# crockwell/far

Measured on AMD Instinct MI355X. Metric: image-pairs/sec (match+solve+regress) at 640x480, higher is better.
Workload: dtype f32

## Files before the change

far_amd/_lib.py:

```python
import ctypes
import os

from . import flags

_HERE = os.path.dirname(os.path.abspath(__file__))
LIB_PATH = flags.value('FAR_HIP_LIB') or os.path.join(_HERE, 'lib', 'libfar_hip.so')

c_p = ctypes.c_void_p
c_i = ctypes.c_int
c_f = ctypes.c_float
c_d = ctypes.c_double
c_sz = ctypes.c_size_t
c_l = ctypes.c_long
c_u32 = ctypes.c_uint32

SIGNATURES = {
    'far_abi_version': (c_i, []),
    'far_last_hip_error': (c_i, []),
    'far_set_tuning': (c_i, [c_i, c_i]),
    'far_mfma_probe_f16': (c_i, [c_i, c_i, c_i, c_p, c_p, c_p]),
    'far_dual_softmax_workspace_bytes': (c_sz, [c_i, c_i, c_i]),
    'far_dual_softmax_stats_f32': (c_i, [c_p, c_p, c_i, c_i, c_i, c_i, c_f, c_f, c_f, c_p, c_p, c_p, c_p, c_p, c_p]),
    'far_coarse_match_f32': (c_i, [c_p, c_p, c_i, c_i, c_i, c_i, c_f, c_f, c_i, c_i, c_i, c_i, c_i, c_f,
                                   c_p, c_p, c_p, c_p, c_p, c_p, c_p, c_p, c_p, c_p, c_p, c_p, c_p, c_p, c_p, c_p]),
# ... 24 lines not shown
    'far_sinkhorn_dense_focal_workspace_bytes': (c_sz, [c_i, c_i, c_i, c_i, c_i, c_i]),
    'far_sinkhorn_dense_focal_f16s': (c_i, [c_p, c_p, c_i, c_i, c_i, c_i, c_p, c_i, c_p, c_p, c_p, c_p, c_p, c_i, c_f, c_f, c_f, c_f,
                                            c_i, c_p, c_p, c_p, c_p]),
    'far_sinkhorn_dense_focal_bwd_f16': (c_i, [c_p, c_p, c_i, c_i, c_i, c_i, c_p, c_i, c_p, c_p, c_p, c_p, c_p, c_i, c_f, c_f, c_f, c_f,
                                               c_i, c_p, c_p, c_p, c_p, c_p, c_p]),
    'far_emm_pv_f32': (c_i, [c_p, c_p, c_p, c_p, c_i, c_i, c_i, c_f, c_p, c_p, c_p, c_p]),
    'far_fine_gather_f32': (c_i, [c_p, c_l, c_l, c_l, c_l, c_i, c_i, c_i, c_p, c_p, c_i, c_i, c_i, c_i, c_p, c_p]),
    'far_fine_scatter_f32': (c_i, [c_p, c_l, c_l, c_l, c_l, c_i, c_i, c_i, c_p, c_p, c_i, c_i, c_i, c_i, c_p, c_p]),
    'far_fine_scatter_det_f32': (c_i, [c_p, c_l, c_l, c_l, c_l, c_i, c_i, c_i, c_p, c_p, c_i, c_i, c_i, c_i, c_i, c_i, c_p, c_p]),
    'far_fine_expect_f32': (c_i, [c_p, c_p, c_i, c_i, c_i, c_p, c_f, c_p, c_p, c_p, c_p, c_p]),
    'far_linear_attention_workspace_bytes': (c_sz, [c_i, c_i, c_i, c_i]),
    'far_linear_attention_f32': (c_i, [c_p, c_p, c_p, c_i, c_i, c_i, c_i, c_i, c_p, c_p, c_f, c_p, c_p, c_p]),
    'far_linear_attention_apply_f32': (c_i, [c_p, c_p, c_i, c_i, c_i, c_i, c_p, c_f, c_p, c_p]),
    'far_full_attention_workspace_bytes': (c_sz, [c_i, c_i, c_i, c_i, c_i]),
    'far_full_attention_f16s': (c_i, [c_p, c_p, c_p, c_i, c_i, c_i, c_i, c_i, c_p, c_p, c_i, c_p, c_p, c_p, c_p]),
    'far_full_attention_train_f16s': (c_i, [c_p, c_p, c_p, c_i, c_i, c_i, c_i, c_i, c_p, c_p, c_i, c_p, c_p, c_p, c_p, c_p]),
    'far_full_attention_bwd_workspace_bytes': (c_sz, [c_i, c_i, c_i, c_i, c_i]),
    'far_full_attention_bwd_f16s': (c_i, [c_p, c_p, c_p, c_p, c_p, c_p, c_i, c_i, c_i, c_i, c_i, c_p, c_p, c_i, c_p, c_p, c_p, c_p, c_p, c_p]),
    'far_vit_attention_f16s': (c_i, [c_p, c_p, c_p, c_i, c_i, c_i, c_i, c_i, c_l, c_l, c_l, c_l, c_l, c_l, c_i, c_p, c_p, c_p]),
    'far_vit_attention_f16': (c_i, [c_p, c_p, c_p, c_i, c_i, c_i, c_i, c_i, c_l, c_l, c_l, c_l, c_l, c_l, c_i, c_p, c_p, c_p]),
    'far_vit_attention_train_f16s': (c_i, [c_p, c_p, c_p, c_i, c_i, c_i, c_i, c_i, c_l, c_l, c_l, c_l, c_l, c_l, c_i, c_p, c_p, c_p, c_p]),
    'far_vit_attention_bwd_workspace_bytes': (c_sz, [c_i, c_i, c_i, c_i, c_i]),
    'far_vit_attention_bwd_f16s': (c_i, [c_p] * 6 + [c_i] * 5 + [c_l] * 6 + [c_i, c_p, c_p, c_p] + [c_l] * 6 + [c_p, c_p, c_p]),
    'far_linear_attention_bwd_workspace_bytes': (c_sz, [c_i, c_i, c_i, c_i, c_i]),
    'far_linear_attention_bwd_f32': (c_i, [c_p, c_p, c_p, c_p, c_i, c_i, c_i, c_i, c_i, c_p, c_p, c_f, c_p, c_p, c_p, c_p, c_p]),
    'far_layernorm_f32': (c_i, [c_p, c_p, c_p, c_p, c_l, c_i, c_f, c_p, c_p]),
    'far_layernorm_bwd_ws_bytes': (c_l, [c_l, c_i]),
    'far_layernorm_bwd_f32': (c_i, [c_p, c_p, c_p, c_l, c_i, c_f, c_p, c_p, c_p, c_p, c_l, c_p]),
    'far_attn_block_packed_bytes': (c_sz, [c_i]),
    'far_attn_block_f16s': (c_i, [c_p, c_p, c_p, c_l, c_i, c_i, c_i, c_i, c_f, c_f, c_f, c_f, c_f, c_p, c_p, c_f, c_p, c_p, c_p]),
    'far_mlp_fused_packed_bytes': (c_sz, [c_i]),
    'far_mlp_fused_f16s': (c_i, [c_p, c_p, c_p, c_l, c_i, c_f, c_f, c_p, c_p, c_f, c_p, c_p, c_p]),
    'far_mlp_fused_f16': (c_i, [c_p, c_p, c_p, c_l, c_i, c_f, c_f, c_p, c_p, c_f, c_p, c_p, c_p]),
    'far_attn_block_f16': (c_i, [c_p, c_p, c_p, c_l, c_i, c_i, c_i, c_i, c_f, c_f, c_f, c_f, c_f, c_p, c_p, c_f, c_p, c_p, c_p]),
    'far_affine_act_f32': (c_i, [c_p, c_p, c_p, c_p, c_l, c_i, c_l, c_i, c_i, c_f, c_p, c_p]),
    'far_upsample2x_add_f32': (c_i, [c_p, c_p, c_i, c_i, c_i, c_i, c_i, c_p, c_p]),
    'far_upsample2x_bwd_f32': (c_i, [c_p, c_i, c_i, c_i, c_i, c_p, c_p]),
    'far_adamw_table_bytes': (c_l, [c_i, c_l]),
    'far_adamw_step_f32': (c_i, [c_p, c_i, c_l] + [ctypes.c_double] * 7 + [c_p]),
    'far_grad_norm_workspace_bytes': (c_sz, [c_l]),
    'far_grad_norm_f32': (c_i, [c_p, c_i, c_l, c_l, c_l, c_d, c_d, c_i, c_p, c_p]),
    'far_grad_clip_scale_f32': (c_i, [c_p, c_i, c_l, c_p, c_p]),
    'far_adam_step_f32': (c_i, [c_p, c_i, c_l] + [c_d] * 7 + [c_i, c_p, c_i, c_p]),
    'far_prior_from_pose_f32': (c_i, [c_p, c_p, c_p, c_i, c_p, c_p]),
    'far_bn_train_ws_bytes': (c_l, [c_l, c_i]),
    'far_bn_act_train_fwd_f32': (c_i, [c_p, c_p, c_l, c_i, c_p, c_p, c_f, c_f, c_p, c_p, c_i, c_f, c_p, c_p, c_p, c_l, c_p]),
    'far_bn_train_stats_f32': (c_i, [c_p, c_l, c_i, c_p, c_p, c_f, c_f, c_p, c_p, c_p, c_p, c_p, c_p, c_p, c_l, c_p]),
    'far_bn_train_bwd_f32': (c_i, [c_p, c_p, c_p, c_p, c_p, c_p, c_l, c_i, c_i, c_f, c_p, c_p, c_p, c_p, c_p, c_l, c_p]),
    'far_bn_sync_moments_f32': (c_i, [c_p, c_l, c_i, c_p, c_p, c_l, c_p]),
    'far_bn_sync_stats_f32': (c_i, [c_p, c_i, c_i, c_p, c_p, c_f, c_f, c_p, c_p, c_p, c_p]),
    'far_bn_sync_apply_f32': (c_i, [c_p, c_p, c_l, c_i, c_p, c_i, c_f, c_p, c_p]),
    'far_bn_sync_bwd_sums_f32': (c_i, [c_p, c_p, c_p, c_p, c_l, c_i, c_i, c_f, c_p, c_p, c_p, c_p, c_l, c_p]),
    'far_bn_sync_bwd_dx_f32': (c_i, [c_p, c_p, c_p, c_p, c_p, c_p, c_i, c_l, c_i, c_i, c_f, c_p, c_p, c_p, c_p]),
    'far_conv_packed_bytes': (c_sz, [c_i, c_i, c_i, c_i, c_i]),
    'far_conv_pack_f32': (c_i, [c_p, c_i, c_i, c_i, c_i, c_i, c_i, c_p, c_p]),
    'far_weight_scale_f32': (c_i, [c_p, c_l, c_p, c_p]),
    'far_conv_pack_view_f32': (c_i, [c_p, c_l, c_l, c_l, c_i, c_i, c_i, c_i, c_i, c_p, c_p, c_p]),
    'far_enc_layer_saved_floats': (c_l, [c_p]),
    'far_enc_layer_grads_floats': (c_l, [c_p]),
    'far_enc_layer_fwd_ws_bytes': (c_l, [c_p]),
    'far_enc_layer_bwd_ws_bytes': (c_l, [c_p]),
    'far_enc_layer_grads_offsets': (c_i, [c_p, c_p]),
    'far_enc_layer_fwd': (c_i, [c_p, c_p, c_p, c_p, c_p, c_p, c_l, c_p]),
    'far_enc_layer_bwd': (c_i, [c_p, c_p, c_p, c_p, c_p, c_p, c_p, c_l, c_p]),
    'far_stream_fork': (c_p, [c_p, c_i]),
    'far_stream_join': (c_i, [c_p, c_i]),
# ... 133 lines not shown
```

far_amd/flags.py:

```python
import os
from collections import namedtuple

Switch = namedtuple('Switch', 'env module attr off_value neutral scope doc')
SWITCHES = [
    Switch('FAR_NO_WINO', 'far_amd.ops', 'USE_WINO', False, 'parity', 'inference',
           'stride-1 3x3 convolutions on K9 (direct implicit GEMM) instead of K17 (Winograd F(2x2,3x3)); same operator, other summation'),
    Switch('FAR_NO_PAD', 'far_amd.loftr.backbone', 'PAD_CHANNELS', False, 'bitwise', 'inference',
           'the 196-channel backbone maps stored with 196 channels instead of 208 (zero weights for the extra ones: exact zeros)'),
    Switch('FAR_NO_PREFETCH', 'far_amd.loftr.model:LoFTR', 'head_prefetch', False, 'bitwise', 'inference',
           "the head's feature stage computed inside forward_rt_prediction instead of enqueued behind K1"),
    Switch('FAR_NO_SIDE_STREAM', 'far_amd.loftr.model:LoFTR', 'head_side_stream', False, 'bitwise', 'inference',
           "the head's feature stage on the step's own stream behind K1 (rounds 2-5) instead of on a second stream next to K1 and the fine level"),
    Switch('FAR_FPN_STREAM', 'far_amd.loftr.model:LoFTR', 'fpn_side_stream', True, 'bitwise', 'inference',
           "OPT-IN (1 switches it ON; default off): the FPN's fine branch on a side stream next to the coarse transformer and K1 (-0.6 ms per 32 "
           "pairs; off by default because the roofline launch -- K17 208 -> 208 @ 240x320 -- then shares the GPU and its in-step duration "
           "in a kernel trace is no longer its own)"),
    Switch('FAR_NO_GATHER_FUSE', 'far_amd.loftr.stages:FinePreprocess', 'fused_gather', False, 'bitwise', 'inference',
           'FinePreprocess.merge_feat on a materialised window tensor (K3 gather + K9) instead of K9 reading through the match indices'),
    Switch('FAR_NO_KV', 'far_amd.loftr.transformer:LoFTREncoderLayer', 'fused_kv', False, 'parity', 'inference',
           "k, v projections + K5's first half as separate launches instead of K9's k|v epilogue (the K'^T V sum changes order)"),
    Switch('FAR_NO_QAPPLY', 'far_amd.loftr.transformer:LoFTREncoderLayer', 'fused_apply', False, 'parity', 'inference',
           "q projection + K5's second half as separate launches instead of K9's attention-apply epilogue (q no longer stays in split operands)"),
    Switch('FAR_NO_STACK', 'far_amd.loftr.transformer:LocalFeatureTransformer', 'stack_self', False, 'bitwise', 'inference',
           "the two 'self' calls of an encoder layer on the two images separately instead of one call on both"),
    Switch('FAR_NO_BN', 'far_amd.ops', 'USE_HIP_BATCHNORM_TRAIN', False, 'parity', 'training',
           'training-mode BatchNorm on nn.BatchNorm2d + torch activations instead of K19 (tests/test_train_kernels_gpu.py holds K19 to the module)'),
]

ENV_ONLY = {
    'FAR_HIP_LIB': ('load', 'path of another build of libfar_hip.so (tools/ab_build.py: same-box A/B against a git revision); skips the build-id check'),
    'FAR_TUNING': ('load', 'comma-separated key=value pairs handed to far_set_tuning at load time, e.g. FAR_TUNING="10=1,8=1" (keys below)'),
    'FAR_SKIP_ASM_CHECK': ('build', "1: far_amd/build.py does not scan the generated code (K9's asm pixel loads; the LDS-DMA ring rule of every kernel with global_load_lds; the half-register writes of the asm fp16 split) after recompiling"),
    'FAR_EXTRA_HIPCC_FLAGS': ('build', 'extra hipcc flags of an experiment build (-DFAR_WINO_EXP=..., tools/wino_exp.sh); part of the build id'),
    'FAR_COMMIT': ('tools', 'commit stamp tools/collect_profiles.sh / tools/step_floors.py write into the profile files'),
    'FAR_C3_PY_NODE': ('bench', "bench.py --workload c3: the encoder layer's autograd node driven from Python instead of far_enc_layer_fwd / _bwd"),
    'FAR_C3_NO_OVERLAP': ('bench', 'bench.py --workload c3: the layer node without side streams'),
    'FAR_C3_PER_OP': ('bench', 'bench.py --workload c3: one autograd node per operator instead of per layer'),
    'FAR_TORCH_ADAMW': ('bench', 'bench.py --workload c3: torch.optim.AdamW instead of K20'),
    'FAR_CUDNN_BENCHMARK': ('bench', 'bench.py: torch.backends.cudnn.benchmark for the vendor comparison legs'),
}

Tuning = namedtuple('Tuning', 'key default values neutral doc')
TUNING = [
    Tuning(0, 3, (0, 1, 2, 4, 7), 'bitwise', 'bit mask of exact-f32 kernels that stagger wave-slot priorities: 1 k_stats, 2 k_match, 4 k_emm_pv'),
    Tuning(1, 0, (1,), 'parity', 'K1 exact-f32 variant: the other tile shape (another summation order of the row statistics)'),
    Tuning(2, 0, (1,), 'bitwise', 'conf_matrix writer variant A (store pattern)'),
    Tuning(3, 0, (1,), 'bitwise', 'conf_matrix writer variant B (store pattern)'),
    Tuning(4, 0, (1,), 'bitwise', 'K9 without the seven-tile mode / K5 windows on the generic path'),
    Tuning(5, 0, (1, 2, 4), 'bitwise', 'K5 apply: tiles per unit'),
    Tuning(6, 0, (64, 256), 'parity', "K5: tokens per K'^T V chunk (another partial-sum grouping)"),
    Tuning(7, 0, (1,), 'bitwise', 'K9 Linear launches always on full-height tiles'),
    Tuning(8, 0, (1,), 'bitwise', 'K17 splits its operands with the five-instruction split2 instead of v_fma_mix (same values)'),
    Tuning(9, 0, (1,), 'bitwise', 'K17 runs a short last channel block on the full body'),
    Tuning(10, 0, (1,), 'bitwise', "K1's match pass without the tile prescreen"),
    Tuning(11, 0, (1, 2), 'bitwise', "K14's pipeline: 0 = 4 waves / 3 slots / counted waits, two workgroups per CU; 1 = 8 waves / 4 slots / counted, one per CU (round 5's form); 2 = 4 waves / 3 slots / vmcnt(0) per phase (fallback without a wait table)"),
# ... 33 lines not shown
```

far_amd/loftr/transformer.py:

```python
import copy
import os
from functools import partial

import torch
import torch.nn as nn

from .. import _vendor as ag
from .. import flags, ops
from ..pose6d import pose_mean_6d, pose_std_6d


class LinearAttention(nn.Module):

    def __init__(self, eps=1e-6, use_num_corres=False):
        super().__init__()
        self.eps = eps
        self.use_num_corres = use_num_corres

    def forward(self, queries, keys, values, q_mask=None, kv_mask=None, loftr_preds=None):
        N, L, H, D = queries.shape
        S = keys.shape[1]
        if ag.needs_grad(queries, keys, values):
            if queries.is_cuda and D in (16, 32):
                return ops.linear_attention_train(queries.reshape(N, L, H * D), keys.reshape(N, S, H * D),
# ... 12 lines not shown

    def __init__(self, use_dropout=False, attention_dropout=0.1, use_num_corres=False):
        super().__init__()
        self.use_dropout = use_dropout
        self.attention_dropout = attention_dropout
        self.use_num_corres = use_num_corres

    def forward(self, queries, keys, values, q_mask=None, kv_mask=None, loftr_preds=None):
        N, L, H, D = queries.shape
        S = keys.shape[1]
        if self.training and self.use_dropout:
            raise NotImplementedError('FullAttention: dropout inside the softmax attention core is not built')
        if ag.needs_grad(queries, keys, values):
            if not self.full_training:
                raise NotImplementedError('FullAttention: training / gradients through the softmax attention core are off for this '
                                          'module (inference only); LoFTR.set_full_attention_training() / full_training = True '
                                          'turns the HIP backward on')
            return ops.full_attention_train(queries.reshape(N, L, H * D), keys.reshape(N, S, H * D), values.reshape(N, S, H * D), H,
                                            q_mask, kv_mask).view(N, L, H, D)
        out = ops.full_attention(queries.reshape(N, L, H * D).contiguous(), keys.reshape(N, S, H * D).contiguous(),
                                 values.reshape(N, S, H * D).contiguous(), H, q_mask, kv_mask)
        return out.view(N, L, H, D)


class LoFTREncoderLayer(nn.Module):
    split_operands = True
    dense_split = True
    hip_training = True
    full_training = False
    layer_node = True
    overlap = True
    native_node = True
    fused_mlp = True
    fused_attn = True
    fused_apply = not flags.off('FAR_NO_QAPPLY')
    fused_kv = not flags.off('FAR_NO_KV')

    def __init__(self, d_model, nhead, attention='linear', use_num_corres=False):
        super().__init__()
        if attention not in ('linear', 'full'):
            raise NotImplementedError(f"attention={attention!r}: only 'linear' (the FAR configuration) and 'full' have kernels")
        self.full = attention == 'full'
        self.dim = d_model // nhead
        self.nhead = nhead
        self.q_proj = nn.Linear(d_model, d_model, bias=False)
        self.k_proj = nn.Linear(d_model, d_model, bias=False)
        self.v_proj = nn.Linear(d_model, d_model, bias=False)
        self.attention = FullAttention(use_num_corres=use_num_corres) if self.full else LinearAttention(use_num_corres=use_num_corres)
        self.merge = nn.Linear(d_model, d_model, bias=False)
        self.mlp = nn.Sequential(
            nn.Linear(d_model * 2, d_model * 2, bias=False),
            nn.ReLU(True),
            nn.Linear(d_model * 2, d_model, bias=False),
        )
        self.norm1 = nn.LayerNorm(d_model)
        self.norm2 = nn.LayerNorm(d_model)

    def forward(self, x, source, x_mask=None, source_mask=None, loftr_preds=None, out=None):
        bs = x.size(0)
        if self.full and x.is_cuda and ag.needs_grad(x, source, self.norm1.weight) and not self.full_training:
            raise NotImplementedError("LoFTREncoderLayer(attention='full'): training / gradients through the softmax attention core "
                                      'are off for this layer (inference only); LoFTR.set_full_attention_training() / '
                                      'full_training = True turns the HIP backward on')
        if self.full and not x.is_cuda:
            raise ops._lib.FarHipError("LoFTREncoderLayer(attention='full') needs tensors on the GPU (no CPU fallback exists)")
        if ag.needs_grad(x, source, self.norm1.weight) or not x.is_cuda:
# ... 36 lines not shown
            h = ops.linear_f16s(x, lin('mlp0', self.mlp[0]), act='relu', x2=msg)
            return ops.linear_f16s(h, lin('mlp2', self.mlp[2]), ln=(self.norm2.weight, self.norm2.bias, self.norm2.eps),
                                   post_residual=x, out=out)
        if (not self.full and self.fused_kv and x.shape[-1] == 256 and self.nhead == 8 and source.shape[1] >= 64 and x_mask is None
                and source_mask is None):
            pkv = pk.get(('kv-state', sp), [self.k_proj.weight, self.v_proj.weight],
                         lambda: ops.PackedConv(ops.kv_interleaved_weight(self.k_proj.weight, self.v_proj.weight, self.nhead), split=sp))
            S = source.shape[1]
            if self.fused_apply and x.shape[1] >= 64:
                _, image = ops.linear_kv_state(source, pkv, S, want_image=True)
                msg = ops.linear_q_apply(x, lin('q', self.q_proj), image, S, eps=self.attention.eps)
            else:
                kv = ops.linear_kv_state(source, pkv, S)
                q = ops.linear_f16s(x, lin('q', self.q_proj))
                msg = ops.linear_attention_apply(q, kv, self.nhead, S, eps=self.attention.eps)
        else:
            if fuse and source is x:
                q, k, v = ops.linear_f16s(x, lin('qkv', self.q_proj, self.k_proj, self.v_proj), out_planes=3)
            elif fuse:
                q = ops.linear_f16s(x, lin('q', self.q_proj))
                k, v = ops.linear_f16s(source, lin('kv', self.k_proj, self.v_proj), out_planes=2)
            else:
                q = ops.linear_f16s(x, lin('q', self.q_proj))
                k = ops.linear_f16s(source, lin('k', self.k_proj))
                v = ops.linear_f16s(source, lin('v', self.v_proj))
            q, k, v = heads(q), heads(k), heads(v)
            msg = self.attention(q, k, v, q_mask=x_mask, kv_mask=source_mask, loftr_preds=loftr_preds)
        msg = ops.linear_f16s(msg.view(bs, -1, self.nhead * self.dim), lin('merge', self.merge, sp=spd),
                              ln=(self.norm1.weight, self.norm1.bias, self.norm1.eps))
        if self.fused_mlp and x.shape[-1] == 128:
            pm = pk.get(('mlp-fused',), [self.mlp[0].weight, self.mlp[2].weight],
                        lambda: ops.PackedMlp(self.mlp[0].weight, self.mlp[2].weight))
            return ops.mlp_fused(x, msg.contiguous(), pm, self.norm2.weight, self.norm2.bias, self.norm2.eps, out=out, plain16=not sp)
        h = ops.linear_f16s(x, lin('mlp0', self.mlp[0], sp=spd), act='relu', x2=msg)
        return ops.linear_f16s(h, lin('mlp2', self.mlp[2], sp=spd), ln=(self.norm2.weight, self.norm2.bias, self.norm2.eps),
                               post_residual=x, out=out)


def _halves_of_one_buffer(a, b):
    return (a.is_contiguous() and b.is_contiguous() and a.shape == b.shape and
            a.untyped_storage().data_ptr() == b.untyped_storage().data_ptr() and b.storage_offset() == a.storage_offset() + a.numel())


class LocalFeatureTransformer(nn.Module):
    stack_self = not flags.off('FAR_NO_STACK')

    def __init__(self, config):
        super().__init__()
        self.config = config
        self.d_model = config['d_model']
        self.nhead = config['nhead']
        self.layer_names = config['layer_names']
        if 'regress_use_num_corres' not in config:
            config['regress_use_num_corres'] = False
        layer = LoFTREncoderLayer(config['d_model'], config['nhead'], config['attention'],
                                  config['regress_use_num_corres'])
        self.layers = nn.ModuleList([copy.deepcopy(layer) for _ in range(len(self.layer_names))])
        for p in self.parameters():
            if p.dim() > 1:
                nn.init.xavier_uniform_(p)

    def forward(self, feat0, feat1, mask0=None, mask1=None, loftr_preds=None, inv_loftr_preds=None, joint_out=False):
        assert self.d_model == feat0.size(2), "the feature number of src and transformer must be equal"
        joint_out = joint_out and feat0.is_cuda and feat0.shape == feat1.shape and not ag.needs_grad(feat0, feat1)
        n = feat0.size(0)
        last = len(self.layers) - 1
# ... 358 lines not shown
```

far_amd/ops/fine.py:

```python
import ctypes
import os
import threading

import torch

from .. import _lib, flags
from ._base import _CONV_ACT_EXP, _p, _stream, _written, overflow_flag


def fine_gather(feat_f, b_ids, cell_ids, wc, W, stride, out=None):
    lib = _lib.load()
    M = int(b_ids.shape[0])
    N, C, Hf, Wf = feat_f.shape
    if out is None:
        out = torch.empty(M, W * W, C, dtype=torch.float32, device=feat_f.device)
    elif tuple(out.shape) != (M, W * W, C) or not out.is_contiguous() or out.dtype != torch.float32:
        raise _lib.FarHipError('fine_gather: `out` must be a contiguous fp32 (M, W*W, C) tensor')
    if M == 0:
        return out
    if not feat_f.is_cuda or feat_f.dtype != torch.float32:
        raise _lib.FarHipError('fine_gather needs an fp32 GPU feature map')
    sn, sc, sh, sw = feat_f.stride()
    rc = lib.far_fine_gather_f32(ctypes.c_void_p(feat_f.data_ptr()), sn, sc, sh, sw, C, Hf, Wf,
                                 _p(b_ids, torch.int64), _p(cell_ids, torch.int64), int(wc), int(W), int(stride), M,
# ... 83 lines not shown
        self.e0, self.e2 = exp_of(w0), exp_of(w2)
        ar = lambda n: torch.arange(n, device=dev)
        s_, t_, l_, e_ = ar(16).view(16, 1, 1, 1), ar(8).view(1, 8, 1, 1), ar(64).view(1, 1, 64, 1), ar(8).view(1, 1, 1, 8)
        hc = 32 * t_ + (l_ & 31)
        k = 32 * (s_ >> 1) + 16 * (l_ >> 5) + 8 * (s_ & 1) + e_
        g1 = planes(w0[hc.expand(16, 8, 64, 8), k.expand(16, 8, 64, 8)] * 2.0 ** self.e0)
        g1 = g1.permute(1, 2, 0, 3, 4).contiguous()
        t2, u2, c2, l2, e2 = (ar(8).view(8, 1, 1, 1, 1), ar(2).view(1, 2, 1, 1, 1), ar(4).view(1, 1, 4, 1, 1),
                              ar(64).view(1, 1, 1, 64, 1), ar(8).view(1, 1, 1, 1, 8))
        co = 32 * c2 + (l2 & 31)
        hk = 32 * t2 + 16 * u2 + 4 * (l2 >> 5) + (e2 & 3) + 8 * (e2 >> 2)
        shp = (8, 2, 4, 64, 8)
        g2 = planes(w2[co.expand(shp), hk.expand(shp)] * 2.0 ** self.e2)
        g2 = g2.permute(1, 2, 3, 0, 4, 5).contiguous()
        self.packed = torch.cat([g1.reshape(-1), g2.reshape(-1)]).view(torch.uint8)
        assert self.packed.numel() == lib.far_mlp_fused_packed_bytes(d)
        self.d = d
        self.hscale = 2.0 ** -self.e0
        self.oscale = 2.0 ** -(self.e2 + _CONV_ACT_EXP)

def mlp_fused(x, msg, pack, gamma, beta, eps, out=None, plain16=False):
    lib = _lib.load()
    if x.shape != msg.shape or x.shape[-1] != pack.d:
        raise _lib.FarHipError('mlp_fused: x and msg must both be (..., 128)')
    R = x.numel() // pack.d
    y = torch.empty_like(x) if out is None else out
    name = 'far_mlp_fused_f16' if plain16 else 'far_mlp_fused_f16s'
    rc = getattr(lib, name)(_p(x, torch.float32), _p(msg, torch.float32), _p(pack.packed), R, pack.d, pack.hscale, pack.oscale,
                            _p(gamma, torch.float32), _p(beta, torch.float32), float(eps), _p(y, torch.float32),
                            _p(overflow_flag(x.device)), _stream())
    _lib.check(rc, name)
    return y if out is None else _written(y)

class PackedAttn:

    def __init__(self, wq, wk, wv, wm):
        lib = _lib.load()
        ws = [w.detach().float() for w in (wk, wv, wq, wm)]
        d = ws[0].shape[0]
        if any(tuple(w.shape) != (d, d) for w in ws) or lib.far_attn_block_packed_bytes(d) == 0:
            raise _lib.FarHipError('far_attn_block_f16s is built for d_model = 128')
        dev = ws[0].device

        def exp_of(w):
            amax = float(w.abs().max())
            return 14 - (torch.frexp(torch.tensor(amax)).exponent.item() if amax > 0 else 0)

        def planes(v):
            hi = v.half()
            return torch.stack([hi, (v - hi.float()).half()])

        self.exps = [exp_of(w) for w in ws]
        ar = lambda n: torch.arange(n, device=dev)
        c_, k_, t_, l_, e_ = (ar(4).view(4, 1, 1, 1, 1), ar(2).view(1, 2, 1, 1, 1), ar(4).view(1, 1, 4, 1, 1),
                              ar(64).view(1, 1, 1, 64, 1), ar(8).view(1, 1, 1, 1, 8))
        shp = (4, 2, 4, 64, 8)
        co = (32 * t_ + (l_ & 31)).expand(shp)
        ci = (32 * c_ + 16 * (l_ >> 5) + 8 * k_ + e_).expand(shp)

        def proj(w, ex):
            return planes(w[co, ci] * 2.0 ** ex).permute(1, 2, 3, 0, 4, 5).contiguous()

        pk, pv, pq = proj(ws[0], self.exps[0]), proj(ws[1], self.exps[1]), proj(ws[2], self.exps[2])
        kvi = torch.stack([pk, pv], 1).reshape(-1)
        mi = (32 * c_ + 16 * k_ + 4 * (l_ >> 5) + (e_ & 3) + 8 * (e_ >> 2)).expand(shp)
        pm = planes(ws[3][co, mi] * 2.0 ** self.exps[3]).permute(1, 2, 3, 0, 4, 5).contiguous()
# ... 20 lines not shown
```

include/far_hip.h:

```cpp
#ifndef FAR_HIP_H
#define FAR_HIP_H

#include <stddef.h>
#include <stdint.h>

#ifdef __cplusplus
extern "C" {
#endif

typedef struct ihipStream_t* far_stream_t;

int far_abi_version(void);
const char* far_build_id(void);
int far_last_hip_error(void);
int far_set_tuning(int key, int value);

void* far_stream_fork(far_stream_t main, int i);
int far_stream_join(far_stream_t main, int i);

int far_mfma_probe_f16(int mode, int iters, int rounds, float* sink, double* flops_out, far_stream_t stream);


size_t far_dual_softmax_workspace_bytes(int Z, int L, int S);

// ... 166 lines not shown
typedef struct far_enc_layer {
    long bs, L, S;
    int C, nhead, self_attn, split, act_exp, overlap;
    float eps1, eps2, attn_eps;
    const void* img[6];
    const float* img_scale[6];
    const void* imgT[6];
    const float* imgT_scale[6];
    const float *g1, *b1, *g2, *b2;
    int* overflow;
} far_enc_layer;
long far_enc_layer_saved_floats(const far_enc_layer* d);
long far_enc_layer_grads_floats(const far_enc_layer* d);
long far_enc_layer_fwd_ws_bytes(const far_enc_layer* d);
long far_enc_layer_bwd_ws_bytes(const far_enc_layer* d);
int far_enc_layer_grads_offsets(const far_enc_layer* d, long* out12);
int far_enc_layer_fwd(const far_enc_layer* d, const float* x, const float* source, float* saved, float* y, void* ws, long ws_bytes,
                      far_stream_t stream);
int far_enc_layer_bwd(const far_enc_layer* d, const float* x, const float* source, const float* saved, const float* gy, float* grads,
                      void* ws, long ws_bytes, far_stream_t stream);

size_t far_attn_block_packed_bytes(int d_model);
int far_attn_block_f16s(const float* x, const float* src, const void* packed, long nwin, int L, int S, int d_model, int heads,
                        float scale_k, float scale_v, float scale_q, float scale_m, float attn_eps, const float* gamma,
                        const float* beta, float ln_eps, float* out, int* overflow, far_stream_t stream);
size_t far_mlp_fused_packed_bytes(int d_model);
int far_mlp_fused_f16s(const float* x, const float* msg, const void* packed, long R, int d_model, float hscale, float oscale,
                       const float* gamma, const float* beta, float eps, float* out, int* overflow, far_stream_t stream);
int far_attn_block_f16(const float* x, const float* src, const void* packed, long nwin, int L, int S, int d_model, int heads,
                       float scale_k, float scale_v, float scale_q, float scale_m, float attn_eps, const float* gamma,
                       const float* beta, float ln_eps, float* out, int* overflow, far_stream_t stream);
int far_mlp_fused_f16(const float* x, const float* msg, const void* packed, long R, int d_model, float hscale, float oscale,
                      const float* gamma, const float* beta, float eps, float* out, int* overflow, far_stream_t stream);


int far_affine_act_f32(const float* x, const float* scale, const float* shift, const float* res, long N, int C,
                       long HW, int nhwc, int act, float slope, float* y, far_stream_t stream);

int far_upsample2x_add_f32(const float* lo, const float* hi, int N, int h, int w, int C, int nhwc, float* out,
                           far_stream_t stream);

long far_adamw_table_bytes(int n, long nblocks);
int far_adamw_step_f32(const void* table, int n, long nblocks, double lr, double beta1, double beta2, double eps, double wd, double bc1,
                       double bc2_sqrt, far_stream_t stream);
size_t far_grad_norm_workspace_bytes(long nblocks);
int far_grad_norm_f32(const void* table, int n, long nblocks, long first, long total, double norm_type, double max_norm,
                      int count_skipped, void* workspace, far_stream_t stream);
int far_grad_clip_scale_f32(const void* table, int n, long nblocks, const void* workspace, far_stream_t stream);
int far_adam_step_f32(const void* table, int n, long nblocks, double lr, double beta1, double beta2, double eps, double wd, double bc1,
                      double bc2_sqrt, int coupled, const void* clip_workspace, int skip_nonfinite, far_stream_t stream);

long far_bn_train_ws_bytes(long M, int C);
int far_bn_act_train_fwd_f32(const float* x, const float* res, long M, int C, const float* gamma, const float* beta, float eps,
                             float momentum, float* running_mean, float* running_var, int act, float slope, float* y, float* vec,
                             void* ws, long ws_bytes, far_stream_t stream);
int far_bn_train_stats_f32(const float* x, long M, int C, const float* gamma, const float* beta, float eps, float momentum,
                           float* running_mean, float* running_var, float* scale, float* shift, float* mean_out, float* rstd_out,
                           void* ws, long ws_bytes, far_stream_t stream);
int far_bn_train_bwd_f32(const float* x, const float* dy, const float* y, const float* mean, const float* rstd, const float* gamma,
                         long M, int C, int act, float slope, float* dx, float* dgamma, float* dbeta, float* dres, void* ws,
                         long ws_bytes, far_stream_t stream);

int far_bn_sync_moments_f32(const float* x, long M, int C, double* rec, void* ws, long ws_bytes, far_stream_t stream);
int far_bn_sync_stats_f32(const double* recs, int W, int C, const float* gamma, const float* beta, float eps, float momentum,
                          float* running_mean, float* running_var, float* vec, far_stream_t stream);
int far_bn_sync_apply_f32(const float* x, const float* res, long M, int C, const float* vec, int act, float slope, float* y,
// ... 153 lines not shown
```

Before: 379.1.

## Fuse d_model-256 MLP block into one kernel keeping hidden activations on-chip

```diff
diff --git a/far_amd/_lib.py b/far_amd/_lib.py
--- a/far_amd/_lib.py
+++ b/far_amd/_lib.py
@@ -80,6 +80,9 @@
     'far_mlp_fused_packed_bytes': (c_sz, [c_i]),
     'far_mlp_fused_f16s': (c_i, [c_p, c_p, c_p, c_l, c_i, c_f, c_f, c_p, c_p, c_f, c_p, c_p, c_p]),
     'far_mlp_fused_f16': (c_i, [c_p, c_p, c_p, c_l, c_i, c_f, c_f, c_p, c_p, c_f, c_p, c_p, c_p]),
+    'far_mlp256_fused_packed_bytes': (c_sz, []),
+    'far_mlp256_fused_f16s': (c_i, [c_p, c_p, c_p, c_l, c_f, c_f, c_p, c_p, c_f, c_p, c_p, c_p]),
+    'far_mlp256_fused_f16': (c_i, [c_p, c_p, c_p, c_l, c_f, c_f, c_p, c_p, c_f, c_p, c_p, c_p]),
     'far_attn_block_f16': (c_i, [c_p, c_p, c_p, c_l, c_i, c_i, c_i, c_i, c_f, c_f, c_f, c_f, c_f, c_p, c_p, c_f, c_p, c_p, c_p]),
     'far_affine_act_f32': (c_i, [c_p, c_p, c_p, c_p, c_l, c_i, c_l, c_i, c_i, c_f, c_p, c_p]),
     'far_upsample2x_add_f32': (c_i, [c_p, c_p, c_i, c_i, c_i, c_i, c_i, c_p, c_p]),
diff --git a/far_amd/csrc/mlp256_fused_f16s.hip b/far_amd/csrc/mlp256_fused_f16s.hip
--- /dev/null
+++ b/far_amd/csrc/mlp256_fused_f16s.hip
@@ -0,0 +1,298 @@
+#include "common.h"
+
+namespace {
+
+typedef _Float16 f16x8 __attribute__((ext_vector_type(8)));
+typedef __attribute__((address_space(3))) void* lptr_t;
+
+constexpr int DM = 256;
+constexpr int KIN = 2 * DM;
+constexpr int HID = 2 * DM;
+constexpr int HCH = 128;
+constexpr int NCH = HID / HCH;
+constexpr int HT = HCH / 32;
+constexpr int CT = DM / 32;
+constexpr int NS1 = KIN / 32;
+constexpr int NS2 = HCH / 16;
+constexpr int NSC = NS1 + NS2;
+constexpr int SLAB = 16384;
+constexpr int NSLAB = NCH * NSC;
+constexpr int RING = 3;
+constexpr int WAVES = 4;
+constexpr int PIECES = 16 / WAVES;
+constexpr float ACT_SCALE = 16.0f;
+static_assert(NSC % RING == 0, "ring slots are immediates inside the chunk loop");
+
+__device__ __forceinline__ void glds16(const void* gsrc, unsigned lds_dst_uniform) {
+    unsigned keep;
+    asm volatile("s_mov_b32 %0, m0\n\ts_mov_b32 m0, %2\n\ts_nop 0\n\tglobal_load_lds_dwordx4 %1, off\n\ts_mov_b32 m0, %0"
+                 : "=&s"(keep) : "v"(gsrc), "s"(lds_dst_uniform) : "memory");
+}
+
+__device__ __forceinline__ void split8(const float4& u, const float4& v, float scale, f16x8& hi, f16x8& lo) {
+    const float x[8] = {u.x, u.y, u.z, u.w, v.x, v.y, v.z, v.w};
+#pragma unroll
+    for (int i = 0; i < 8; i += 2) {
+        f16x2 h, l;
+        split2(f32x2{x[i], x[i + 1]} * f32x2{scale, scale}, h, l);
+        hi[i] = h.x; hi[i + 1] = h.y;
+        lo[i] = l.x; lo[i + 1] = l.y;
+    }
+}
+
+#define FAR_DPP_F(v, ctrl) __builtin_bit_cast(float, __builtin_amdgcn_update_dpp(0, __builtin_bit_cast(int, v), ctrl, 0xF, 0xF, true))
+__device__ __forceinline__ float sum32(float v) {
+    v += FAR_DPP_F(v, 0xB1);
+    v += FAR_DPP_F(v, 0x4E);
+    v += FAR_DPP_F(v, 0x141);
+    v += FAR_DPP_F(v, 0x140);
+    return v + shfl_xor_f(v, 16);
+}
+
+__device__ __forceinline__ int lane_now() {
+    int l;
+    asm volatile("v_mbcnt_lo_u32_b32 %0, -1, 0\n\tv_mbcnt_hi_u32_b32 %0, -1, %0" : "=v"(l));
+    return l;
+}
+
+
+template <bool SPLIT>
+__global__ __launch_bounds__(256, 2) void k_mlp256(const float* __restrict__ x, const float* __restrict__ msg,
+                                                   const unsigned char* __restrict__ wimg, long R, float hscale, float oscale,
+                                                   const float* __restrict__ gamma, const float* __restrict__ beta, float eps,
+                                                   float* __restrict__ out, int* __restrict__ overflow) {
+    __shared__ __attribute__((aligned(16))) unsigned char lds[RING * SLAB + WAVES * 4096];
+    unsigned char* const ring = lds;
+    unsigned char* const xs = lds + RING * SLAB;
+    const int tid = threadIdx.x, lane = tid & 63, l31 = lane & 31, h = lane >> 5;
+    const int wave = __builtin_amdgcn_readfirstlane(tid >> 6);
+    const long row0 = (long)blockIdx.x * (32 * WAVES) + 32 * wave;
+    const unsigned ring_base = (unsigned)__builtin_amdgcn_readfirstlane((int)(unsigned)(size_t)(lptr_t)ring);
+    const unsigned xs_base = (unsigned)__builtin_amdgcn_readfirstlane((int)(unsigned)(size_t)(lptr_t)(xs + wave * 4096));
+    auto request_w = [&](const unsigned char* chunk_src, int j) {
+        const unsigned dst = ring_base + (unsigned)((j % RING) * SLAB);
+#pragma unroll
+        for (int i = 0; i < PIECES; ++i)
+            glds16(chunk_src + (size_t)j * SLAB + (wave + WAVES * i) * 1024, dst + (wave + WAVES * i) * 1024);
+    };
+    const int rr = lane >> 3, q = lane & 7;
+    const long brow0 = (long)blockIdx.x * (32 * WAVES);
+    const float* xb = x + brow0 * DM;
+    const float* mb = msg + brow0 * DM;
+    unsigned goff[4];
+#pragma unroll
+    for (int j = 0; j < 4; ++j) {
+        const int r = 8 * j + rr;
+        long gr = row0 + r;
+        gr = gr < R ? gr : R - 1;
+        goff[j] = (unsigned)(gr - brow0) * DM + 4 * (q ^ ((r ^ (r >> 3)) & 7));
+    }
+    auto request_x = [&](int c) {
+        const float* base = (c < NS1 / 2 ? xb : mb) + 32 * (c & (NS1 / 2 - 1));
+#pragma unroll
+        for (int j = 0; j < 4; ++j) glds16(base + goff[j], xs_base + j * 1024);
+    };
+    request_x(0);
+    request_w(wimg + (unsigned)lane * 16, 0);
+    request_w(wimg + (unsigned)lane * 16, 1);
+    f32x16 acc1[HT], acc2[CT];
+#pragma unroll
+    for (int t = 0; t < HT; ++t)
+#pragma unroll
+        for (int r = 0; r < 16; ++r) acc1[t][r] = 0.f;
+#pragma unroll
+    for (int ct = 0; ct < CT; ++ct)
+#pragma unroll
+        for (int r = 0; r < 16; ++r) acc2[ct][r] = 0.f;
+    float hid_chk = 0.f;
+    const unsigned char* xrd = xs + wave * 4096 + (l31 >> 3) * 1024 + (l31 & 7) * 128;
+    const int sw = (l31 ^ (l31 >> 3)) & 7;
+
+#pragma unroll 1
+    for (int hc = 0; hc < NCH; ++hc) {
+#pragma unroll
+        for (int j = 0; j < 4; ++j) asm volatile("" : "+v"(goff[j]));
+        const unsigned char* csrc = wimg + (size_t)hc * NSC * SLAB + (unsigned)lane_now() * 16;
+#pragma unroll
+        for (int j = 0; j < NS1; ++j) {
+            asm volatile("s_waitcnt vmcnt(0)" ::: "memory");
+            ring_barrier();
+            f16x8 xh[2], xl[2];
+            {
+                float4 raw[4];
+#pragma unroll
+                for (int i = 0; i < 4; ++i) raw[i] = *reinterpret_cast<const float4*>(xrd + (((2 * h + i + 2 * (i >> 1)) ^ sw) * 16));
+                asm volatile("s_waitcnt lgkmcnt(0)" ::: "memory");
+                if (j + 1 < NS1) request_x(j + 1);
+                split8(raw[0], raw[1], ACT_SCALE, xh[0], xl[0]);
+                split8(raw[2], raw[3], ACT_SCALE, xh[1], xl[1]);
+            }
+            request_w(csrc, j + 2);
+            const unsigned char* slab = ring + (j % RING) * SLAB + lane * 16;
+            f16x8 ah[3], al[3];
+#pragma unroll
+            for (int i = 0; i < 2; ++i) {
+                ah[i] = *reinterpret_cast<const f16x8*>(slab + i * 2048);
+                al[i] = *reinterpret_cast<const f16x8*>(slab + i * 2048 + 1024);
+            }
+#pragma unroll
+            for (int i = 0; i < 2 * HT; ++i) {
+                if (i + 2 < 2 * HT) {
+                    ah[(i + 2) % 3] = *reinterpret_cast<const f16x8*>(slab + (i + 2) * 2048);
+                    al[(i + 2) % 3] = *reinterpret_cast<const f16x8*>(slab + (i + 2) * 2048 + 1024);
+                }
+                const int ks = i / HT, t = i % HT;
+                acc1[t] = __builtin_amdgcn_mfma_f32_32x32x16_f16(ah[i % 3], xh[ks], acc1[t], 0, 0, 0);
+                if (SPLIT) {
+                    acc1[t] = __builtin_amdgcn_mfma_f32_32x32x16_f16(al[i % 3], xh[ks], acc1[t], 0, 0, 0);
+                    acc1[t] = __builtin_amdgcn_mfma_f32_32x32x16_f16(ah[i % 3], xl[ks], acc1[t], 0, 0, 0);
+                }
+                __builtin_amdgcn_sched_group_barrier(0x100, SPLIT ? 2 : 1, 0);
+                __builtin_amdgcn_sched_group_barrier(0x008, SPLIT ? 3 : 1, 0);
+            }
+        }
+#pragma unroll
+        for (int jj = 0; jj < NS2; ++jj) {
+            const int j = NS1 + jj, t = jj >> 1, u = jj & 1;
+            asm volatile("s_waitcnt vmcnt(0)" ::: "memory");
+            ring_barrier();
+            if (j + 2 < NSC) request_w(csrc, j + 2);
+            else if (hc + 1 < NCH) request_w(csrc + (size_t)NSC * SLAB, j + 2 - NSC);
+            if (jj == 0 && hc + 1 < NCH) request_x(0);
+            const unsigned char* slab = ring + (j % RING) * SLAB + lane * 16;
+            f16x8 ha, hl;
+#pragma unroll
+            for (int e = 0; e < 8; e += 2) {
+                hid_chk += acc1[t][8 * u + e] + acc1[t][8 * u + e + 1];
+                const f32x2 hv = __builtin_elementwise_max(f32x2{acc1[t][8 * u + e], acc1[t][8 * u + e + 1]} * f32x2{hscale, hscale}, f32x2{0.f, 0.f});
+                f16x2 h2, l2;
+                split2(hv, h2, l2);
+                ha[e] = h2.x; ha[e + 1] = h2.y;
+                hl[e] = l2.x; hl[e + 1] = l2.y;
+                acc1[t][8 * u + e] = 0.f; acc1[t][8 * u + e + 1] = 0.f;
+            }
+            f16x8 bh[3], bl[3];
+#pragma unroll
+            for (int i = 0; i < 2; ++i) {
+                bh[i] = *reinterpret_cast<const f16x8*>(slab + (i * 2) * 1024);
+                bl[i] = *reinterpret_cast<const f16x8*>(slab + (i * 2 + 1) * 1024);
+            }
+#pragma unroll
+            for (int ct = 0; ct < CT; ++ct) {
+                if (ct + 2 < CT) {
+                    bh[(ct + 2) % 3] = *reinterpret_cast<const f16x8*>(slab + ((ct + 2) * 2) * 1024);
+                    bl[(ct + 2) % 3] = *reinterpret_cast<const f16x8*>(slab + ((ct + 2) * 2 + 1) * 1024);
+                }
+                acc2[ct] = __builtin_amdgcn_mfma_f32_32x32x16_f16(ha, bh[ct % 3], acc2[ct], 0, 0, 0);
+                if (SPLIT) {
+                    acc2[ct] = __builtin_amdgcn_mfma_f32_32x32x16_f16(ha, bl[ct % 3], acc2[ct], 0, 0, 0);
+                    acc2[ct] = __builtin_amdgcn_mfma_f32_32x32x16_f16(hl, bh[ct % 3], acc2[ct], 0, 0, 0);
+                }
+                __builtin_amdgcn_sched_group_barrier(0x100, SPLIT ? 2 : 1, 0);
+                __builtin_amdgcn_sched_group_barrier(0x008, SPLIT ? 3 : 1, 0);
+            }
+        }
+    }
+
+    const int elane = lane_now();
+    if (overflow) {
+        float chk = hid_chk;
+#pragma unroll
+        for (int ct = 0; ct < CT; ++ct)
+#pragma unroll
+            for (int r = 0; r < 16; ++r) chk += acc2[ct][r];
+        if (__any(!(fabsf(chk) <= FLT_MAX)) && elane == 0) atomicOr(overflow, 1);
+    }
+    asm volatile("s_waitcnt vmcnt(0)" ::: "memory");
+    ring_barrier();
+    const int el31 = elane & 31, eh = elane >> 5;
+    float* lw = reinterpret_cast<float*>(lds + wave * 16384);
+    auto put = [&](int half) {
+#pragma unroll
+        for (int c4 = 0; c4 < 4; ++c4)
+#pragma unroll
+            for (int r = 0; r < 16; ++r) lw[mfma32_row(r, eh) * 128 + 32 * c4 + el31] = acc2[4 * half + c4][r] * oscale;
+        asm volatile("s_waitcnt lgkmcnt(0)" ::: "memory");
+    };
+    auto get = [&](int it) { return *reinterpret_cast<const float4*>(lw + (2 * it + eh) * 128 + 4 * el31); };
+    const float inv_c = 1.0f / (float)DM;
+    float part[16], mean[16], rstd[16];
+#pragma unroll
+    for (int half = 0; half < 2; ++half) {
+        put(half);
+#pragma unroll
+        for (int it = 0; it < 16; ++it) {
+            const float4 v = get(it);
+            const float t = sum32((v.x + v.y) + (v.z + v.w));
+            part[it] = half == 0 ? t : part[it] + t;
+        }
+        asm volatile("s_waitcnt lgkmcnt(0)" ::: "memory");
+    }
+#pragma unroll
+    for (int it = 0; it < 16; ++it) mean[it] = part[it] * inv_c;
+#pragma unroll
+    for (int half = 0; half < 2; ++half) {
+        put(half);
+#pragma unroll
+        for (int it = 0; it < 16; ++it) {
+            float4 v = get(it);
+            v.x -= mean[it]; v.y -= mean[it]; v.z -= mean[it]; v.w -= mean[it];
+            const float t = sum32((v.x * v.x + v.y * v.y) + (v.z * v.z + v.w * v.w));
+            part[it] = half == 0 ? t : part[it] + t;
+        }
+        asm volatile("s_waitcnt lgkmcnt(0)" ::: "memory");
+    }
+#pragma unroll
+    for (int it = 0; it < 16; ++it) rstd[it] = 1.0f / sqrtf(part[it] * inv_c + eps);
+#pragma unroll
+    for (int half = 0; half < 2; ++half) {
+        put(half);
+        const int co = 128 * half + 4 * el31;
+        const float4 g4 = *reinterpret_cast<const float4*>(gamma + co), b4 = *reinterpret_cast<const float4*>(beta + co);
+#pragma unroll
+        for (int it = 0; it < 16; ++it) {
+            const long orow = row0 + 2 * it + eh;
+            float4 v = get(it);
+            if (orow < R) {
+                const float4 pr = *reinterpret_cast<const float4*>(x + orow * DM + co);
+                v.x -= mean[it]; v.y -= mean[it]; v.z -= mean[it]; v.w -= mean[it];
+                float4 o;
+                o.x = v.x * rstd[it] * g4.x + b4.x + pr.x; o.y = v.y * rstd[it] * g4.y + b4.y + pr.y;
+                o.z = v.z * rstd[it] * g4.z + b4.z + pr.z; o.w = v.w * rstd[it] * g4.w + b4.w + pr.w;
+                *reinterpret_cast<float4*>(out + orow * DM + co) = o;
+            }
+        }
+        asm volatile("s_waitcnt lgkmcnt(0)" ::: "memory");
+    }
+}
+
+template <bool SPLIT>
+int mlp256_fused_launch(const float* x, const float* msg, const void* packed, long R, float hscale, float oscale,
+                        const float* gamma, const float* beta, float eps, float* out, int* overflow, hipStream_t stream) {
+    far_clear_errors();
+    if (R == 0) return FAR_OK;
+    if (!x || !msg || !packed || !gamma || !beta || !out || R < 0 || out == x || out == msg) return FAR_EINVAL;
+    const long nb = (R + 32 * WAVES - 1) / (32 * WAVES);
+    if (nb > 0x7fffffffL) return FAR_EINVAL;
+    hipLaunchKernelGGL(k_mlp256<SPLIT>, dim3((unsigned)nb), dim3(64 * WAVES), 0, stream, x, msg, (const unsigned char*)packed, R, hscale,
+                       oscale, gamma, beta, eps, out, overflow);
+    return far_check_launch();
+}
+
+}
+
+extern "C" {
+
+size_t far_mlp256_fused_packed_bytes(void) { return (size_t)NSLAB * SLAB; }
+
+int far_mlp256_fused_f16s(const float* x, const float* msg, const void* packed, long R, float hscale, float oscale,
+                          const float* gamma, const float* beta, float eps, float* out, int* overflow, hipStream_t stream) {
+    return mlp256_fused_launch<true>(x, msg, packed, R, hscale, oscale, gamma, beta, eps, out, overflow, stream);
+}
+
+int far_mlp256_fused_f16(const float* x, const float* msg, const void* packed, long R, float hscale, float oscale,
+                         const float* gamma, const float* beta, float eps, float* out, int* overflow, hipStream_t stream) {
+    return mlp256_fused_launch<false>(x, msg, packed, R, hscale, oscale, gamma, beta, eps, out, overflow, stream);
+}
+
+}
diff --git a/far_amd/flags.py b/far_amd/flags.py
--- a/far_amd/flags.py
+++ b/far_amd/flags.py
@@ -21,6 +21,9 @@
            "k, v projections + K5's first half as separate launches instead of K9's k|v epilogue (the K'^T V sum changes order)"),
     Switch('FAR_NO_QAPPLY', 'far_amd.loftr.transformer:LoFTREncoderLayer', 'fused_apply', False, 'parity', 'inference',
            "q projection + K5's second half as separate launches instead of K9's attention-apply epilogue (q no longer stays in split operands)"),
+    Switch('FAR_NO_MLP256', 'far_amd.loftr.transformer:LoFTREncoderLayer', 'fused_mlp256', False, 'parity', 'inference',
+           'the MLP block of the d_model-256 layers as two K9 launches (mlp[0] + ReLU, mlp[2] + norm2 + residual) instead of one K27 launch (launches of 9 600 rows and more: LoFTREncoderLayer.mlp256_min_rows) '
+           '(the hidden tensor goes through memory; K27 sums in K9\'s order throughout: the same bits)'),
     Switch('FAR_NO_STACK', 'far_amd.loftr.transformer:LocalFeatureTransformer', 'stack_self', False, 'bitwise', 'inference',
            "the two 'self' calls of an encoder layer on the two images separately instead of one call on both"),
     Switch('FAR_NO_BN', 'far_amd.ops', 'USE_HIP_BATCHNORM_TRAIN', False, 'parity', 'training',
diff --git a/far_amd/loftr/transformer.py b/far_amd/loftr/transformer.py
--- a/far_amd/loftr/transformer.py
+++ b/far_amd/loftr/transformer.py
@@ -68,6 +68,8 @@
     overlap = True
     native_node = True
     fused_mlp = True
+    fused_mlp256 = not flags.off('FAR_NO_MLP256')
+    mlp256_min_rows = 9600
     fused_attn = True
     fused_apply = not flags.off('FAR_NO_QAPPLY')
     fused_kv = not flags.off('FAR_NO_KV')
@@ -170,6 +172,11 @@
             pm = pk.get(('mlp-fused',), [self.mlp[0].weight, self.mlp[2].weight],
                         lambda: ops.PackedMlp(self.mlp[0].weight, self.mlp[2].weight))
             return ops.mlp_fused(x, msg.contiguous(), pm, self.norm2.weight, self.norm2.bias, self.norm2.eps, out=out, plain16=not sp)
+        if (self.fused_mlp and self.fused_mlp256 and x.shape[-1] == 256 and x.numel() >= 256 * self.mlp256_min_rows
+                and x.dtype == torch.float32 and msg.dtype == torch.float32):
+            pm = pk.get(('mlp256-fused',), [self.mlp[0].weight, self.mlp[2].weight],
+                        lambda: ops.PackedMlp256(self.mlp[0].weight, self.mlp[2].weight))
+            return ops.mlp256_fused(x, msg.contiguous(), pm, self.norm2.weight, self.norm2.bias, self.norm2.eps, out=out, plain16=not spd)
         h = ops.linear_f16s(x, lin('mlp0', self.mlp[0], sp=spd), act='relu', x2=msg)
         return ops.linear_f16s(h, lin('mlp2', self.mlp[2], sp=spd), ln=(self.norm2.weight, self.norm2.bias, self.norm2.eps),
                                post_residual=x, out=out)
diff --git a/far_amd/ops/fine.py b/far_amd/ops/fine.py
--- a/far_amd/ops/fine.py
+++ b/far_amd/ops/fine.py
@@ -139,6 +139,60 @@
     _lib.check(rc, name)
     return y if out is None else _written(y)
 
+class PackedMlp256:
+
+    def __init__(self, w0, w2):
+        lib = _lib.load()
+        w0, w2 = w0.detach().float(), w2.detach().float()
+        d = 256
+        if tuple(w0.shape) != (2 * d, 2 * d) or tuple(w2.shape) != (d, 2 * d):
+            raise _lib.FarHipError(f'far_mlp256_fused_f16s is built for d_model = 256 (got weights {tuple(w0.shape)}, {tuple(w2.shape)})')
+        dev = w0.device
+
+        def exp_of(w):
+            amax = float(w.abs().max())
+            return 14 - (torch.frexp(torch.tensor(amax)).exponent.item() if amax > 0 else 0)
+
+        def planes(v):
+            hi = v.half()
+            return torch.stack([hi, (v - hi.float()).half()])
+
+        self.e0, self.e2 = exp_of(w0), exp_of(w2)
+        ar = lambda n, *shape: torch.arange(n, device=dev).view(*shape)
+        c_, j_, k_, t_, l_, e_ = (ar(4, 4, 1, 1, 1, 1, 1), ar(16, 1, 16, 1, 1, 1, 1), ar(2, 1, 1, 2, 1, 1, 1), ar(4, 1, 1, 1, 4, 1, 1),
+                                  ar(64, 1, 1, 1, 1, 64, 1), ar(8, 1, 1, 1, 1, 1, 8))
+        shp = (4, 16, 2, 4, 64, 8)
+        m_ = l_ & 31
+        hch = (128 * c_ + 32 * t_ + ((m_ & 19) | ((m_ & 4) << 1) | ((m_ & 8) >> 1))).expand(shp)
+        k = (32 * j_ + 16 * k_ + 8 * (l_ >> 5) + e_).expand(shp)
+        g1 = planes(w0[hch, k] * 2.0 ** self.e0)
+        g1 = g1.permute(1, 2, 3, 4, 0, 5, 6).reshape(4, 16 * 8192)
+        c_, t_, u_, o_, l_, e_ = (ar(4, 4, 1, 1, 1, 1, 1), ar(4, 1, 4, 1, 1, 1, 1), ar(2, 1, 1, 2, 1, 1, 1), ar(8, 1, 1, 1, 8, 1, 1),
+                                  ar(64, 1, 1, 1, 1, 64, 1), ar(8, 1, 1, 1, 1, 1, 8))
+        shp = (4, 4, 2, 8, 64, 8)
+        co = (32 * o_ + (l_ & 31)).expand(shp)
+        hk = (128 * c_ + 32 * t_ + 16 * u_ + 8 * (l_ >> 5) + e_).expand(shp)
+        g2 = planes(w2[co, hk] * 2.0 ** self.e2)
+        g2 = g2.permute(1, 2, 3, 4, 0, 5, 6).reshape(4, 8 * 8192)
+        self.packed = torch.cat([g1, g2], 1).contiguous().view(-1).view(torch.uint8)
+        assert self.packed.numel() == lib.far_mlp256_fused_packed_bytes()
+        self.d = d
+        self.hscale = 2.0 ** -self.e0
+        self.oscale = 2.0 ** -(self.e2 + _CONV_ACT_EXP)
+
+def mlp256_fused(x, msg, pack, gamma, beta, eps, out=None, plain16=False):
+    lib = _lib.load()
+    if x.shape != msg.shape or x.shape[-1] != pack.d:
+        raise _lib.FarHipError('mlp256_fused: x and msg must both be (..., 256)')
+    R = x.numel() // pack.d
+    y = torch.empty_like(x) if out is None else out
+    name = 'far_mlp256_fused_f16' if plain16 else 'far_mlp256_fused_f16s'
+    rc = getattr(lib, name)(_p(x, torch.float32), _p(msg, torch.float32), _p(pack.packed), R, pack.hscale, pack.oscale,
+                            _p(gamma, torch.float32), _p(beta, torch.float32), float(eps), _p(y, torch.float32),
+                            _p(overflow_flag(x.device)), _stream())
+    _lib.check(rc, name)
+    return y if out is None else _written(y)
+
 class PackedAttn:
 
     def __init__(self, wq, wk, wv, wm):
diff --git a/include/far_hip.h b/include/far_hip.h
--- a/include/far_hip.h
+++ b/include/far_hip.h
@@ -222,6 +222,12 @@
                        const float* beta, float ln_eps, float* out, int* overflow, far_stream_t stream);
 int far_mlp_fused_f16(const float* x, const float* msg, const void* packed, long R, int d_model, float hscale, float oscale,
                       const float* gamma, const float* beta, float eps, float* out, int* overflow, far_stream_t stream);
+
+size_t far_mlp256_fused_packed_bytes(void);
+int far_mlp256_fused_f16s(const float* x, const float* msg, const void* packed, long R, float hscale, float oscale,
+                          const float* gamma, const float* beta, float eps, float* out, int* overflow, far_stream_t stream);
+int far_mlp256_fused_f16(const float* x, const float* msg, const void* packed, long R, float hscale, float oscale,
+                         const float* gamma, const float* beta, float eps, float* out, int* overflow, far_stream_t stream);
 
 
 int far_affine_act_f32(const float* x, const float* scale, const float* shift, const float* res, long N, int C,
```

New measurement: 382.3, median of 6. Within noise of the previous version (+0.8%).
